# stonkgs/stonkgs

Hardware: AMD Instinct MI355X
Metric: text-triple pairs/sec (whole node), seq_len=512 hidden=768, 1/2/4/8 MI355X (higher is better)
Workload: dtype bf16; 1 GPU; STonKGs-150k pretraining step (12L/768h, V=28996, K=175094), per-GPU batch 64, seq 256 text + 256 entity, dropout 0.1, AdamW lr 1e-4; global_batch=64, seq_len=512, parallelism=dp1

## Files before the change

stonkgs_amd/csrc/loss.hip:

```cpp
#include <atomic>
#include "common.h"
#include "stonk_flags.h"

namespace {

__global__ __launch_bounds__(1024) void label_compact_kernel(const long* __restrict__ labels, long n, int half, int S,
                                                             int offset, int* __restrict__ rows_out,
                                                             int* __restrict__ targets_out, int* __restrict__ count_out,
                                                             const int* __restrict__ row_of_pos) {
  constexpr int R = 16;
  __shared__ unsigned long long ball[R * 16];
  __shared__ int pre[R * 16];
  __shared__ int wtot[4];
  const int t = threadIdx.x, lane = t & 63, w = t >> 6;
  int base = 0;
  for (long c0 = 0; c0 < n; c0 += (long)R * 1024) {
    long lab[R];
#pragma unroll
    for (int j = 0; j < R; ++j) {
      const long i = c0 + j * 1024 + t;
      lab[j] = i < n ? labels[i] : -100;
    }
#pragma unroll
    for (int j = 0; j < R; ++j) {
      const unsigned long long bal = __ballot(lab[j] != -100);
      if (lane == 0) ball[j * 16 + w] = bal;
    }
    __syncthreads();
    int cnt = 0, inc = 0;
    if (t < R * 16) {
      cnt = __popcll(ball[t]);
      inc = cnt;
#pragma unroll
      for (int o = 1; o < 64; o <<= 1) {
        const int v = __shfl_up(inc, o, 64);
        if (lane >= o) inc += v;
      }
      if (lane == 63) wtot[w] = inc;
    }
    __syncthreads();
    if (t < R * 16) {
      int woff = 0;
      for (int k = 0; k < w; ++k) woff += wtot[k];
      pre[t] = woff + inc - cnt;
    }
    __syncthreads();
    const unsigned long long below = (1ULL << lane) - 1ULL;
#pragma unroll
    for (int j = 0; j < R; ++j) {
      if (lab[j] == -100) continue;
      const long i = c0 + j * 1024 + t;
      const int dst = base + pre[j * 16 + w] + __popcll(ball[j * 16 + w] & below);
      const long b = i / half;
      const long pos = b * S + offset + (i - b * half);
      rows_out[dst] = row_of_pos ? row_of_pos[pos] : (int)pos;
      targets_out[dst] = (int)lab[j];
    }
    base += wtot[0] + wtot[1] + wtot[2] + wtot[3];
    __syncthreads();
  }
  if (t == 0) *count_out = base;
}

__global__ __launch_bounds__(256) void gather_rows_kernel(const bf16* __restrict__ src, long ld_src,
                                                          const int* __restrict__ rows, const int* __restrict__ count,
                                                          bf16* __restrict__ dst, long ld_dst, int cols, long cap) {
  const int cnt = *count;
  long lim = ((long)(cnt + 127) / 128) * 128;
  lim = lim < cap ? lim : cap;
  const int nch = cols >> 3;
  const long total = lim * nch;
  for (long i = (long)blockIdx.x * 256 + threadIdx.x; i < total; i += (long)gridDim.x * 256) {
    const long r = i / nch;
    const int c = (int)(i - r * nch);
    bf16x8 v;
#pragma unroll
    for (int j = 0; j < 8; ++j) v[j] = (bf16)0.f;
    if (r < cnt) v = *(const bf16x8*)(src + (long)rows[r] * ld_src + c * 8);
    *(bf16x8*)(dst + r * ld_dst + c * 8) = v;
  }
}

__global__ __launch_bounds__(256) void scatter_rows_kernel(const bf16* __restrict__ src, long ld_src,
                                                           const int* __restrict__ rows, const int* __restrict__ count,
                                                           bf16* __restrict__ dst, long ld_dst, int cols) {
  const int cnt = *count;
  const int nch = cols >> 3;
  const long total = (long)cnt * nch;
  for (long i = (long)blockIdx.x * 256 + threadIdx.x; i < total; i += (long)gridDim.x * 256) {
    const long r = i / nch;
    const int c = (int)(i - r * nch);
    *(bf16x8*)(dst + (long)rows[r] * ld_dst + c * 8) = *(const bf16x8*)(src + r * ld_src + c * 8);
  }
}

__global__ __launch_bounds__(256) void scatter_rows_f32_kernel(const float* __restrict__ src, long ld_src,
                                                               const int* __restrict__ rows,
                                                               const int* __restrict__ count, bf16* __restrict__ dst,
                                                               long ld_dst, int cols) {
  const int cnt = *count;
  const int nch = cols >> 3;
  const long total = (long)cnt * nch;
  for (long i = (long)blockIdx.x * 256 + threadIdx.x; i < total; i += (long)gridDim.x * 256) {
    const long r = i / nch;
    const int c = (int)(i - r * nch);
    const f32x4 a = *(const f32x4*)(src + r * ld_src + c * 8), b = *(const f32x4*)(src + r * ld_src + c * 8 + 4);
    bf16x8 o = {(bf16)a[0], (bf16)a[1], (bf16)a[2], (bf16)a[3], (bf16)b[0], (bf16)b[1], (bf16)b[2], (bf16)b[3]};
    *(bf16x8*)(dst + (long)rows[r] * ld_dst + c * 8) = o;
  }
}

#ifndef STONK_XENT_BLOCKS
#define STONK_XENT_BLOCKS 2048
#endif
constexpr int XENT_POOL = 16;
__device__ float g_xent_part[XENT_POOL][STONK_XENT_BLOCKS];
__device__ unsigned g_xent_ticket[XENT_POOL];
std::atomic<unsigned> g_xent_next{0};

template <typename LT> struct LogitVec;
template <> struct LogitVec<float> {
  static __device__ __forceinline__ void load8(const float* x, float (&v)[8]) {
    const f32x4 a = *(const f32x4*)x, b = *(const f32x4*)(x + 4);
#pragma unroll
    for (int j = 0; j < 4; ++j) { v[j] = a[j]; v[4 + j] = b[j]; }
  }
};
template <> struct LogitVec<_Float16> {
  static __device__ __forceinline__ void load8(const _Float16* x, float (&v)[8]) {
    const f16x8 a = *(const f16x8*)x;
#pragma unroll
    for (int j = 0; j < 8; ++j) v[j] = (float)a[j];
  }
};

template <typename LT>
__global__ __launch_bounds__(256) void softmax_xent_kernel(const LT* __restrict__ logits, long ld, int ncols, int npad,
                                                           const int* __restrict__ targets, const int* __restrict__ count,
                                                           float* __restrict__ loss_sum, bf16* __restrict__ dlogits,
                                                           long ld_d, float gscale, int* __restrict__ err,
                                                           int cap_rows, int slot) {
  __shared__ float red_m[4], red_s[4];
  float own_loss = 0.f;
  const int cnt = *count;
  const int t = threadIdx.x, lane = t & 63, w = t >> 6;
  const float g = gscale / (float)cnt;
  for (int row = blockIdx.x; row < cnt; row += gridDim.x) {
    const LT* x = logits + (long)row * ld;
    float m = -3.0e38f, s = 0.f;
    const int n8 = ncols >> 3;
    for (int i0 = 0; i0 < n8; i0 += 1024) {
      float v[4][8];
#pragma unroll
      for (int u = 0; u < 4; ++u) {
        const int i = i0 + 256 * u + t;
        if (i < n8) {
          LogitVec<LT>::load8(x + 8 * i, v[u]);
        } else {
#pragma unroll
          for (int j = 0; j < 8; ++j) v[u][j] = -__builtin_inff();
        }
      }
      float vm = v[0][0];
#pragma unroll
      for (int u = 0; u < 4; ++u)
#pragma unroll
        for (int j = 0; j < 8; ++j) vm = fmaxf(vm, v[u][j]);
      if (vm > m) {
        s *= __expf(m - vm);
        m = vm;
      }
#pragma unroll
      for (int u = 0; u < 4; ++u)
#pragma unroll
        for (int j = 0; j < 8; ++j) s += __expf(v[u][j] - m);
    }
    for (int i = (n8 << 3) + t; i < ncols; i += 256) {
      const float v = (float)x[i];
      if (v > m) {
        s *= __expf(m - v);
        m = v;
      }
      s += __expf(v - m);
    }
#pragma unroll
    for (int o = 32; o > 0; o >>= 1) {
      const float m2 = __shfl_xor(m, o, 64), s2 = __shfl_xor(s, o, 64);
      const float mn = fmaxf(m, m2);
      s = s * __expf(m - mn) + s2 * __expf(m2 - mn);
      m = mn;
    }
    if (lane == 0) {
      red_m[w] = m;
      red_s[w] = s;
    }
    __syncthreads();
    float M = fmaxf(fmaxf(red_m[0], red_m[1]), fmaxf(red_m[2], red_m[3]));
    float Ssum = 0.f;
#pragma unroll
    for (int j = 0; j < 4; ++j) Ssum += red_s[j] * __expf(red_m[j] - M);
    const float lse = M + __logf(Ssum);
    int tgt = targets[row];
    if (tgt < 0 || tgt >= ncols) {
      if (t == 0) atomicOr(err, 8);
      tgt = 0;
    }
    if (t == 0) own_loss += lse - (float)x[tgt];
    if (dlogits) {
      bf16* d = dlogits + (long)row * ld_d;
      const int p8 = npad >> 3, f8 = ncols >> 3;
      const float nlse = -lse;
      for (int i0 = 0; i0 < f8; i0 += 1024) {
        float v[4][8];
#pragma unroll
        for (int u = 0; u < 4; ++u) {
          const int i = i0 + 256 * u + t;
          if (i < f8) LogitVec<LT>::load8(x + 8 * i, v[u]);
        }
#pragma unroll
        for (int u = 0; u < 4; ++u) {
          const int i = i0 + 256 * u + t;
          if (i >= f8) continue;
          const int c0 = i * 8;
          float pr[8];
#pragma unroll
          for (int j = 0; j < 8; ++j) pr[j] = __expf(v[u][j] + nlse);
          if (tgt >= c0 && tgt < c0 + 8) {
#pragma unroll
            for (int j = 0; j < 8; ++j)
              if (c0 + j == tgt) pr[j] -= 1.f;
          }
          bf16x8 o;
#pragma unroll
          for (int j = 0; j < 8; ++j) o[j] = (bf16)(pr[j] * g);
          *(bf16x8*)(d + c0) = o;
        }
      }
      for (int i = f8 + t; i < p8; i += 256) {
        const int c0 = i * 8;
        bf16x8 o;
#pragma unroll
        for (int j = 0; j < 8; ++j) {
          float pr = 0.f;
          if (c0 + j < ncols) {
            pr = __expf((float)x[c0 + j] - lse);
            if (c0 + j == tgt) pr -= 1.f;
          }
          o[j] = (bf16)(pr * g);
        }
        *(bf16x8*)(d + c0) = o;
      }
    }
    __syncthreads();
  }
  if (dlogits) {
    const int lim = (cnt + 63) / 64 * 64;
    for (int row = cnt + blockIdx.x; row < lim && row < cap_rows; row += gridDim.x) {
      bf16* d = dlogits + (long)row * ld_d;
      bf16x8 z;
#pragma unroll
      for (int j = 0; j < 8; ++j) z[j] = (bf16)0.f;
      for (int i = t; i < (npad >> 3); i += 256) *(bf16x8*)(d + i * 8) = z;
    }
  }
  float* part = g_xent_part[slot];
  unsigned* ticket = &g_xent_ticket[slot];
  __shared__ bool last;
  __shared__ double wide[256];
  if (t == 0) {
    (void)__hip_atomic_exchange(&part[blockIdx.x], own_loss, __ATOMIC_RELAXED, __HIP_MEMORY_SCOPE_AGENT);
    asm volatile("s_waitcnt vmcnt(0)" ::: "memory");
    last = __hip_atomic_fetch_add(ticket, 1u, __ATOMIC_RELAXED, __HIP_MEMORY_SCOPE_AGENT) == gridDim.x - 1;
  }
  __syncthreads();
  if (!last) return;
  double tot = 0.0;
  for (int i = t; i < (int)gridDim.x; i += 256)
    tot += (double)__hip_atomic_load(&part[i], __ATOMIC_RELAXED, __HIP_MEMORY_SCOPE_AGENT);
  wide[t] = tot;
  __syncthreads();
  for (int o = 128; o > 0; o >>= 1) {
    if (t < o) wide[t] += wide[t + o];
    __syncthreads();
  }
  if (t == 0) {
    if (cnt > 0) atomicAdd(loss_sum, (float)wide[0]);
    __hip_atomic_store(ticket, 0u, __ATOMIC_RELAXED, __HIP_MEMORY_SCOPE_AGENT);
  }
}

__global__ __launch_bounds__(256) void nsp_xent_kernel(const float* __restrict__ logits, const long* __restrict__ labels,
                                                       int B, int C, float* __restrict__ loss_sum,
                                                       float* __restrict__ dlogits, float gscale, int* __restrict__ err) {
  float local = 0.f;
  int cnt = 0;
  for (int i = 0; i < B; ++i) cnt += labels[i] != -100;
  for (int b = blockIdx.x * 256 + threadIdx.x; b < B; b += gridDim.x * 256) {
    const float* x = logits + (long)b * C;
    long tgt = labels[b];
    float m = x[0];
    for (int c = 1; c < C; ++c) m = fmaxf(m, x[c]);
    float s = 0.f;
    for (int c = 0; c < C; ++c) s += __expf(x[c] - m);
    const float lse = m + __logf(s);
    const bool ignored = tgt == -100;
    if (!ignored && (tgt < 0 || tgt >= C)) {
      atomicOr(err, 16);
      tgt = 0;
    }
    if (!ignored) local += lse - x[tgt];
    if (dlogits)
      for (int c = 0; c < C; ++c)
        dlogits[(long)b * C + c] = ignored ? 0.f : (__expf(x[c] - lse) - (c == tgt ? 1.f : 0.f)) * gscale / (float)cnt;
  }
  local = wave_sum(local);
  if ((threadIdx.x & 63) == 0 && local != 0.f) atomicAdd(loss_sum, local);
  if (blockIdx.x == 0 && threadIdx.x == 0) atomicAdd(loss_sum + 1, (float)cnt);
}

__global__ void loss_finalize_kernel(const float* text_sum, const int* text_cnt, const float* ent_sum, const int* ent_cnt,
                                     const float* nsp_sum_cnt, float* loss_out) {
  const float lt = *text_sum / (float)*text_cnt;
  const float le = *ent_sum / (float)*ent_cnt;
  const float ln = nsp_sum_cnt[0] / nsp_sum_cnt[1];
  loss_out[0] = lt + le + ln;
  loss_out[1] = lt;
  loss_out[2] = le;
  loss_out[3] = ln;
}

}

extern "C" int stonk_label_compact(const int64_t* labels, int64_t n, int half, int S, int offset, int* rows_out,
                                   int* targets_out, int* count_out, const int* row_of_pos, void* stream) {
  STONK_CHECK_ARG(labels && rows_out && targets_out && count_out, STONK_EINVAL);
  STONK_CHECK_ARG(n >= 0 && half > 0 && S >= half && offset >= 0, STONK_ESHAPE);
  hipLaunchKernelGGL(label_compact_kernel, dim3(1), dim3(1024), 0, (hipStream_t)stream, (const long*)labels, (long)n,
                     half, S, offset, rows_out, targets_out, count_out, row_of_pos);
  return stonk_launch_status();
}

extern "C" int stonk_gather_rows_bf16(const void* src, int64_t ld_src, const int* rows, const int* count_dev, void* dst,
                                      int64_t ld_dst, int cols, int64_t cap, void* stream) {
  STONK_CHECK_ARG(src && rows && count_dev && dst, STONK_EINVAL);
  STONK_CHECK_ARG(cols > 0 && cols % 8 == 0 && ld_src % 8 == 0 && ld_dst % 8 == 0 && cap >= 0, STONK_EALIGN);
  if (cap == 0) return STONK_OK;
  hipLaunchKernelGGL(gather_rows_kernel, dim3(1024), dim3(256), 0, (hipStream_t)stream, (const bf16*)src, (long)ld_src,
                     rows, count_dev, (bf16*)dst, (long)ld_dst, cols, (long)cap);
  return stonk_launch_status();
}

extern "C" int stonk_scatter_rows_bf16(const void* src, int64_t ld_src, const int* rows, const int* count_dev,
                                       void* dst, int64_t ld_dst, int cols, void* stream) {
  STONK_CHECK_ARG(src && rows && count_dev && dst, STONK_EINVAL);
  STONK_CHECK_ARG(cols > 0 && cols % 8 == 0 && ld_src % 8 == 0 && ld_dst % 8 == 0, STONK_EALIGN);
  hipLaunchKernelGGL(scatter_rows_kernel, dim3(1024), dim3(256), 0, (hipStream_t)stream, (const bf16*)src, (long)ld_src,
                     rows, count_dev, (bf16*)dst, (long)ld_dst, cols);
  return stonk_launch_status();
}

extern "C" int stonk_scatter_rows_f32_to_bf16(const float* src, int64_t ld_src, const int* rows, const int* count_dev,
                                             void* dst, int64_t ld_dst, int cols, void* stream) {
  STONK_CHECK_ARG(src && rows && count_dev && dst, STONK_EINVAL);
  STONK_CHECK_ARG(cols > 0 && cols % 8 == 0 && ld_src % 4 == 0 && ld_dst % 8 == 0, STONK_EALIGN);
  hipLaunchKernelGGL(scatter_rows_f32_kernel, dim3(1024), dim3(256), 0, (hipStream_t)stream, src, (long)ld_src, rows,
                     count_dev, (bf16*)dst, (long)ld_dst, cols);
  return stonk_launch_status();
}

extern "C" int stonk_softmax_xent_fwd_bwd(const float* logits, int64_t ld, int ncols, int npad, const int* targets,
                                          const int* count_dev, float* loss_sum, void* dlogits, int64_t ld_d,
                                          float grad_scale, int cap_rows, int* err_flag, void* stream) {
  STONK_CHECK_ARG(logits && targets && count_dev && loss_sum && err_flag && cap_rows >= 0, STONK_EINVAL);
  STONK_CHECK_ARG(ncols > 0 && npad >= ncols && npad % 8 == 0 && ld >= npad && ld % 4 == 0, STONK_ESHAPE);
  STONK_CHECK_ARG(!dlogits || (ld_d >= npad && ld_d % 8 == 0), STONK_ESHAPE);
  hipLaunchKernelGGL(softmax_xent_kernel<float>, dim3(STONK_XENT_BLOCKS), dim3(256), 0, (hipStream_t)stream, logits, (long)ld, ncols,
                     npad, targets, count_dev, loss_sum, (bf16*)dlogits, (long)ld_d, grad_scale, err_flag, cap_rows,
                     (int)(g_xent_next.fetch_add(1) % XENT_POOL));
  return stonk_launch_status();
}

extern "C" int stonk_softmax_xent_f16_fwd_bwd(const void* logits_f16, int64_t ld, int ncols, int npad, const int* targets,
                                              const int* count_dev, float* loss_sum, void* dlogits, int64_t ld_d,
                                              float grad_scale, int cap_rows, int* err_flag, void* stream) {
  STONK_CHECK_ARG(logits_f16 && targets && count_dev && loss_sum && err_flag && cap_rows >= 0, STONK_EINVAL);
  STONK_CHECK_ARG(ncols > 0 && npad >= ncols && npad % 8 == 0 && ld >= npad && ld % 8 == 0, STONK_ESHAPE);
  STONK_CHECK_ARG(!dlogits || (ld_d >= npad && ld_d % 8 == 0), STONK_ESHAPE);
  STONK_CHECK_ARG((uintptr_t)logits_f16 % 16 == 0, STONK_EALIGN);
  hipLaunchKernelGGL(softmax_xent_kernel<_Float16>, dim3(STONK_XENT_BLOCKS), dim3(256), 0, (hipStream_t)stream,
                     (const _Float16*)logits_f16, (long)ld, ncols, npad, targets, count_dev, loss_sum, (bf16*)dlogits,
                     (long)ld_d, grad_scale, err_flag, cap_rows,
                     (int)(g_xent_next.fetch_add(1) % XENT_POOL));
  return stonk_launch_status();
}

extern "C" int stonk_nsp_xent_fwd_bwd(const float* logits, const int64_t* labels, int B, int C, float* loss_sum_cnt,
                                      float* dlogits, float grad_scale, int* err_flag, void* stream) {
  STONK_CHECK_ARG(logits && labels && loss_sum_cnt && err_flag, STONK_EINVAL);
  STONK_CHECK_ARG(B > 0 && C > 0 && C <= 64, STONK_ESHAPE);
  hipLaunchKernelGGL(nsp_xent_kernel, dim3((B + 255) / 256), dim3(256), 0, (hipStream_t)stream, logits,
                     (const long*)labels, B, C, loss_sum_cnt, dlogits, grad_scale, err_flag);
  return stonk_launch_status();
}

extern "C" int stonk_loss_finalize(const float* text_sum, const int* text_cnt, const float* ent_sum, const int* ent_cnt,
                                   const float* nsp_sum_cnt, float* loss_out, void* stream) {
  STONK_CHECK_ARG(text_sum && text_cnt && ent_sum && ent_cnt && nsp_sum_cnt && loss_out, STONK_EINVAL);
  hipLaunchKernelGGL(loss_finalize_kernel, dim3(1), dim3(1), 0, (hipStream_t)stream, text_sum, text_cnt, ent_sum, ent_cnt,
                     nsp_sum_cnt, loss_out);
  return stonk_launch_status();
}
```

Measured before the change: 2526 pairs/s.

## Add register/LDS-resident single-pass softmax cross-entropy kernel for f16 logits

Adds a resident softmax-xent kernel that loads each logit row once into registers (and LDS for the larger entity vocabulary) and computes max, sum-exp and gradients from that held copy instead of re-reading the row from global memory several times. Small vocabularies (text, V≈29k) use 256-thread blocks with 16 register pieces. The large entity vocabulary (K≈175k) uses 1024-thread blocks with 14 register pieces plus 8 LDS pieces, launched with one block per CU. The shared epilogue is factored into a helper. This trades much higher register and LDS use, and lower occupancy, for fewer global memory reads.

```diff
diff --git a/stonkgs_amd/csrc/loss.hip b/stonkgs_amd/csrc/loss.hip
--- a/stonkgs_amd/csrc/loss.hip
+++ b/stonkgs_amd/csrc/loss.hip
@@ -133,6 +133,48 @@
     for (int j = 0; j < 8; ++j) v[j] = (float)a[j];
   }
 };
+
+template <int T>
+__device__ __forceinline__ void xent_finish(int cnt, float own_loss, float* __restrict__ loss_sum, bf16* __restrict__ dlogits,
+                                            long ld_d, int npad, int cap_rows, int slot) {
+  const int t = threadIdx.x;
+  if (dlogits) {
+    const int lim = (cnt + 63) / 64 * 64;
+    for (int row = cnt + blockIdx.x; row < lim && row < cap_rows; row += gridDim.x) {
+      bf16* d = dlogits + (long)row * ld_d;
+      bf16x8 z;
+#pragma unroll
+      for (int j = 0; j < 8; ++j) z[j] = (bf16)0.f;
+      for (int i = t; i < (npad >> 3); i += T) *(bf16x8*)(d + i * 8) = z;
+    }
+  }
+  float* part = g_xent_part[slot];
+  unsigned* ticket = &g_xent_ticket[slot];
+  __shared__ bool last;
+  __shared__ double wide[256];
+  if (t == 0) {
+    (void)__hip_atomic_exchange(&part[blockIdx.x], own_loss, __ATOMIC_RELAXED, __HIP_MEMORY_SCOPE_AGENT);
+    asm volatile("s_waitcnt vmcnt(0)" ::: "memory");
+    last = __hip_atomic_fetch_add(ticket, 1u, __ATOMIC_RELAXED, __HIP_MEMORY_SCOPE_AGENT) == gridDim.x - 1;
+  }
+  __syncthreads();
+  if (!last) return;
+  if (t < 256) {
+    double tot = 0.0;
+    for (int i = t; i < (int)gridDim.x; i += 256)
+      tot += (double)__hip_atomic_load(&part[i], __ATOMIC_RELAXED, __HIP_MEMORY_SCOPE_AGENT);
+    wide[t] = tot;
+  }
+  __syncthreads();
+  for (int o = 128; o > 0; o >>= 1) {
+    if (t < o) wide[t] += wide[t + o];
+    __syncthreads();
+  }
+  if (t == 0) {
+    if (cnt > 0) atomicAdd(loss_sum, (float)wide[0]);
+    __hip_atomic_store(ticket, 0u, __ATOMIC_RELAXED, __HIP_MEMORY_SCOPE_AGENT);
+  }
+}
 
 template <typename LT>
 __global__ __launch_bounds__(256) void softmax_xent_kernel(const LT* __restrict__ logits, long ld, int ncols, int npad,
@@ -253,40 +295,142 @@
     }
     __syncthreads();
   }
-  if (dlogits) {
-    const int lim = (cnt + 63) / 64 * 64;
-    for (int row = cnt + blockIdx.x; row < lim && row < cap_rows; row += gridDim.x) {
+  xent_finish<256>(cnt, own_loss, loss_sum, dlogits, ld_d, npad, cap_rows, slot);
+}
+
+typedef __attribute__((ext_vector_type(4))) unsigned piece_t;
+
+template <int T, int NR, int NL>
+__global__ __launch_bounds__(T, 4) void softmax_xent_resident_kernel(const _Float16* __restrict__ logits, long ld, int ncols,
+                                                                  int npad, const int* __restrict__ targets,
+                                                                  const int* __restrict__ count, float* __restrict__ loss_sum,
+                                                                  bf16* __restrict__ dlogits, long ld_d, float gscale,
+                                                                  int* __restrict__ err, int cap_rows, int slot) {
+  extern __shared__ __attribute__((aligned(16))) piece_t held[];
+  constexpr int W = T / 64;
+  __shared__ float red_m[W], red_s[W], tgt_logit;
+  float own_loss = 0.f;
+  const int cnt = *count;
+  const int t = threadIdx.x, lane = t & 63, w = t >> 6;
+  const float g = gscale / (float)cnt;
+  const int np = (ncols + 7) >> 3, rem = ncols & 7;
+  const int ul = (np - 1) / T, tl = (np - 1) % T;
+  const bool in_last = t <= tl, tail_mine = rem != 0 && t == tl;
+  auto holds = [&](int u) { return u < ul || (u == ul && in_last); };
+  const piece_t ninf = {0xFC00FC00u, 0xFC00FC00u, 0xFC00FC00u, 0xFC00FC00u};
+  auto fetch = [&](const _Float16* x, int u) -> piece_t {
+    piece_t v = ninf;
+    if (holds(u)) v = *(const piece_t*)((const char*)x + (unsigned)((u * T + t) * 16));
+    return v;
+  };
+  auto cut_tail = [&](piece_t v) -> piece_t {
+    f16x8 h = __builtin_bit_cast(f16x8, v);
+#pragma unroll
+    for (int j = 1; j < 8; ++j)
+      if (j >= rem) h[j] = -(_Float16)__builtin_inff();
+    return __builtin_bit_cast(piece_t, h);
+  };
+  for (int row = blockIdx.x; row < cnt; row += gridDim.x) {
+    const _Float16* x = logits + (long)row * ld;
+    int tgt = targets[row];
+    if (tgt < 0 || tgt >= ncols) {
+      if (t == 0) atomicOr(err, 8);
+      tgt = 0;
+    }
+    const int ut = (tgt >> 3) / T, tj = tgt & 7;
+    const bool tgt_mine = t == (tgt >> 3) % T;
+    piece_t r[NR > 0 ? NR : 1];
+    if constexpr (NL > 0) {
+      piece_t v[NL];
+#pragma unroll
+      for (int u = 0; u < NL; ++u) v[u] = fetch(x, NR + u);
+#pragma unroll
+      for (int u = 0; u < NR; ++u) r[u] = fetch(x, u);
+#pragma unroll
+      for (int u = 0; u < NL; ++u) {
+        if (NR + u == ul && tail_mine) v[u] = cut_tail(v[u]);
+        held[u * T + t] = v[u];
+      }
+    } else {
+#pragma unroll
+      for (int u = 0; u < NR; ++u) r[u] = fetch(x, u);
+    }
+#pragma unroll
+    for (int u = 0; u < NR; ++u)
+      if (u == ul && tail_mine) r[u] = cut_tail(r[u]);
+    f16x8 hm = __builtin_bit_cast(f16x8, ninf);
+#pragma unroll
+    for (int u = 0; u < NR; ++u) hm = __builtin_elementwise_max(hm, __builtin_bit_cast(f16x8, r[u]));
+#pragma unroll
+    for (int u = 0; u < NL; ++u)
+      if (NR + u <= ul) hm = __builtin_elementwise_max(hm, __builtin_bit_cast(f16x8, held[u * T + t]));
+    float m = (float)hm[0];
+#pragma unroll
+    for (int j = 1; j < 8; ++j) m = fmaxf(m, (float)hm[j]);
+    m = wave_max(m);
+    if (lane == 0) red_m[w] = m;
+    __syncthreads();
+    float M = red_m[0];
+#pragma unroll
+    for (int j = 1; j < W; ++j) M = fmaxf(M, red_m[j]);
+    float s = 0.f;
+    auto sum_piece = [&](piece_t pv, int u) {
+      if (!holds(u)) return;
+      const f16x8 v = __builtin_bit_cast(f16x8, pv);
+#pragma unroll
+      for (int j = 0; j < 8; ++j) s += __expf((float)v[j] - M);
+      if (u == ut && tgt_mine) {
+        float xt = (float)v[0];
+#pragma unroll
+        for (int j = 1; j < 8; ++j)
+          if (j == tj) xt = (float)v[j];
+        tgt_logit = xt;
+      }
+    };
+#pragma unroll
+    for (int u = 0; u < NR; ++u) sum_piece(r[u], u);
+#pragma unroll
+    for (int u = 0; u < NL; ++u)
+      if (NR + u <= ul) sum_piece(held[u * T + t], NR + u);
+    s = wave_sum(s);
+    if (lane == 0) red_s[w] = s;
+    __syncthreads();
+    float Ssum = 0.f;
+#pragma unroll
+    for (int j = 0; j < W; ++j) Ssum += red_s[j];
+    const float lse = M + __logf(Ssum);
+    if (t == 0) own_loss += lse - tgt_logit;
+    if (dlogits) {
       bf16* d = dlogits + (long)row * ld_d;
+      const float nlse = -lse;
+      auto write_piece = [&](piece_t pv, int u) {
+        if (!holds(u)) return;
+        const f16x8 v = __builtin_bit_cast(f16x8, pv);
+        float pr[8];
+#pragma unroll
+        for (int j = 0; j < 8; ++j) pr[j] = __expf((float)v[j] + nlse);
+        if (u == ut && tgt_mine) {
+#pragma unroll
+          for (int j = 0; j < 8; ++j)
+            if (j == tj) pr[j] -= 1.f;
+        }
+        bf16x8 o;
+#pragma unroll
+        for (int j = 0; j < 8; ++j) o[j] = (bf16)(pr[j] * g);
+        *(bf16x8*)(d + 8 * (long)(u * T + t)) = o;
+      };
+#pragma unroll
+      for (int u = 0; u < NR; ++u) write_piece(r[u], u);
+#pragma unroll
+      for (int u = 0; u < NL; ++u)
+        if (NR + u <= ul) write_piece(held[u * T + t], NR + u);
       bf16x8 z;
 #pragma unroll
       for (int j = 0; j < 8; ++j) z[j] = (bf16)0.f;
-      for (int i = t; i < (npad >> 3); i += 256) *(bf16x8*)(d + i * 8) = z;
-    }
-  }
-  float* part = g_xent_part[slot];
-  unsigned* ticket = &g_xent_ticket[slot];
-  __shared__ bool last;
-  __shared__ double wide[256];
-  if (t == 0) {
-    (void)__hip_atomic_exchange(&part[blockIdx.x], own_loss, __ATOMIC_RELAXED, __HIP_MEMORY_SCOPE_AGENT);
-    asm volatile("s_waitcnt vmcnt(0)" ::: "memory");
-    last = __hip_atomic_fetch_add(ticket, 1u, __ATOMIC_RELAXED, __HIP_MEMORY_SCOPE_AGENT) == gridDim.x - 1;
-  }
-  __syncthreads();
-  if (!last) return;
-  double tot = 0.0;
-  for (int i = t; i < (int)gridDim.x; i += 256)
-    tot += (double)__hip_atomic_load(&part[i], __ATOMIC_RELAXED, __HIP_MEMORY_SCOPE_AGENT);
-  wide[t] = tot;
-  __syncthreads();
-  for (int o = 128; o > 0; o >>= 1) {
-    if (t < o) wide[t] += wide[t + o];
-    __syncthreads();
-  }
-  if (t == 0) {
-    if (cnt > 0) atomicAdd(loss_sum, (float)wide[0]);
-    __hip_atomic_store(ticket, 0u, __ATOMIC_RELAXED, __HIP_MEMORY_SCOPE_AGENT);
-  }
+      for (int i = np + t; i < (npad >> 3); i += T) *(bf16x8*)(d + 8 * (long)i) = z;
+    }
+  }
+  xent_finish<T>(cnt, own_loss, loss_sum, dlogits, ld_d, npad, cap_rows, slot);
 }
 
 __global__ __launch_bounds__(256) void nsp_xent_kernel(const float* __restrict__ logits, const long* __restrict__ labels,
@@ -329,6 +473,35 @@
   loss_out[3] = ln;
 }
 
+int xent_cu_count() {
+  static int n_cu = 0;
+  if (n_cu == 0) {
+    int dev = 0;
+    hipDeviceProp_t prop;
+    n_cu = hipGetDevice(&dev) == hipSuccess && hipGetDeviceProperties(&prop, dev) == hipSuccess ? prop.multiProcessorCount : 256;
+    n_cu = n_cu < 1 ? 1 : n_cu > STONK_XENT_BLOCKS ? STONK_XENT_BLOCKS : n_cu;
+  }
+  return n_cu;
+}
+
+template <int T, int NR, int NL>
+int launch_xent_resident(int grid, const void* logits_f16, int64_t ld, int ncols, int npad, const int* targets,
+                         const int* count_dev, float* loss_sum, void* dlogits, int64_t ld_d, float grad_scale, int cap_rows,
+                         int* err_flag, void* stream) {
+  constexpr int LDS = NL * T * 16;
+  static bool attr_done = LDS <= 65536;
+  if (!attr_done) {
+    const hipError_t e = hipFuncSetAttribute((const void*)softmax_xent_resident_kernel<T, NR, NL>,
+                                             hipFuncAttributeMaxDynamicSharedMemorySize, LDS);
+    if (e != hipSuccess) return (int)e;
+    attr_done = true;
+  }
+  hipLaunchKernelGGL((softmax_xent_resident_kernel<T, NR, NL>), dim3(grid), dim3(T), LDS, (hipStream_t)stream,
+                     (const _Float16*)logits_f16, (long)ld, ncols, npad, targets, count_dev, loss_sum, (bf16*)dlogits,
+                     (long)ld_d, grad_scale, err_flag, cap_rows, (int)(g_xent_next.fetch_add(1) % XENT_POOL));
+  return stonk_launch_status();
+}
+
 }
 
 extern "C" int stonk_label_compact(const int64_t* labels, int64_t n, int half, int S, int offset, int* rows_out,
@@ -387,6 +560,13 @@
   STONK_CHECK_ARG(ncols > 0 && npad >= ncols && npad % 8 == 0 && ld >= npad && ld % 8 == 0, STONK_ESHAPE);
   STONK_CHECK_ARG(!dlogits || (ld_d >= npad && ld_d % 8 == 0), STONK_ESHAPE);
   STONK_CHECK_ARG((uintptr_t)logits_f16 % 16 == 0, STONK_EALIGN);
+  const int np = (ncols + 7) / 8;
+  if (np <= 256 * 16)
+    return launch_xent_resident<256, 16, 0>(STONK_XENT_BLOCKS, logits_f16, ld, ncols, npad, targets, count_dev, loss_sum,
+                                            dlogits, ld_d, grad_scale, cap_rows, err_flag, stream);
+  if (np <= 1024 * 22)
+    return launch_xent_resident<1024, 14, 8>(xent_cu_count(), logits_f16, ld, ncols, npad, targets, count_dev, loss_sum,
+                                             dlogits, ld_d, grad_scale, cap_rows, err_flag, stream);
   hipLaunchKernelGGL(softmax_xent_kernel<_Float16>, dim3(STONK_XENT_BLOCKS), dim3(256), 0, (hipStream_t)stream,
                      (const _Float16*)logits_f16, (long)ld, ncols, npad, targets, count_dev, loss_sum, (bf16*)dlogits,
                      (long)ld_d, grad_scale, err_flag, cap_rows,
```

After: 2540 pairs/s, median of 6. No clear change (+0.6%).
